# lvrcek/GNNome-assembly

Measured on AMD Instinct MI355X. Metric: GatedGCN edges/sec fwd+bwd, chr19 assembly graph, higher is better.
Workload: dtype f32 (f16x2 split products, f32 accumulate)

## Files before the change

### gnnome_assembly_amd/csrc/gnm_fused.hip

```cpp
#include <string.h>
#include <type_traits>

#include "gnm_common.h"
#include "gnm_tr.h"

namespace gnm {

typedef float floatx16 __attribute__((ext_vector_type(16)));

constexpr int FH = 128;
constexpr int FTR = 64;
constexpr int FP = FH + 4;
constexpr int FKQ = FH / 8;

using full_t = std::true_type;
using ragged_t = std::false_type;

__global__ void pack_w_k(const float* __restrict__ W, int64_t ld, int ncb, int nn, float* __restrict__ Wp) {
  const int total = ncb * FKQ * 64;
  for (int idx = blockIdx.x * blockDim.x + threadIdx.x; idx < total; idx += gridDim.x * blockDim.x) {
    const int lane = idx & 63, q = (idx >> 6) % FKQ, cb = idx / (64 * FKQ);
    const int i = lane & 31, g = lane >> 5;
    float v[4];
#pragma unroll
// ... 210 lines not shown
    for (int c = 0; c < BKC; ++c) {
      h16x8 n0[2], n1[2];
#pragma unroll
      for (int s = 0; s < 2; ++s) {
        n0[s] = a0[s];
        n1[s] = a1[s];
        if (c + 1 < BKC) {
          n0[s] = *reinterpret_cast<const h16x8*>(p0 + s * BIMG + 16 * (c + 1));
          n1[s] = *reinterpret_cast<const h16x8*>(p1 + s * BIMG + 16 * (c + 1));
        }
      }
      __builtin_amdgcn_sched_barrier(0);
      mfh(acc0, a0[1], f.w[c][0]); mfh(acc1, a1[1], f.w[c][0]);
      mfh(acc0, a0[0], f.w[c][1]); mfh(acc1, a1[0], f.w[c][1]);
      mfh(acc0, a0[0], f.w[c][0]); mfh(acc1, a1[0], f.w[c][0]);
#pragma unroll
      for (int s = 0; s < 2; ++s) { a0[s] = n0[s]; a1[s] = n1[s]; }
      __builtin_amdgcn_sched_barrier(0);
    }
  }
};

template <class MM>
__device__ __forceinline__ float stage_row(void* img, int row, int c4, const float4& v) {
  if constexpr (MM::kScaled) return MM::stage(img, row, c4, v);
  else { MM::stage(img, row, c4, v); return 1.f; }
}

__device__ __forceinline__ void h2_stage_nn(void* img, int row, int c4, const float4& v, int* eref, float* fs, bool first,
                                            bool writer) {
  const unsigned mb = row32_max_bits(max_abs4_bits(v));
  int e = (int)(mb >> 23) & 0xff;
  e = e < 16 ? 16 : e;
  const int eo = first ? e : *eref;
  const int en = e > eo ? e : eo;
  if (writer) {
    *eref = en;
    const int fe = 127 + eo - en;
    *fs = __int_as_float((fe < 0 ? 0 : fe) << 23);
  }
  h16x4 hi, lo;
  split2(v, __int_as_float((268 - en) << 23), hi, lo);
  _Float16* b = reinterpret_cast<_Float16*>(img) + row * BP + c4;
  *reinterpret_cast<h16x4*>(b) = hi;
  *reinterpret_cast<h16x4*>(b + BIMG) = lo;
}
__device__ __forceinline__ void acc_rescale_rows(floatx16& acc, const float* fs, int lg) {
#pragma unroll
  for (int q = 0; q < 4; ++q) {
    const float4 f = ld4(fs + 8 * q + 4 * lg);
    acc[4 * q + 0] *= f.x; acc[4 * q + 1] *= f.y; acc[4 * q + 2] *= f.z; acc[4 * q + 3] *= f.w;
  }
}
__device__ __forceinline__ float h2_ref_inv(int eref) { return __int_as_float((eref - 14) << 23); }

__device__ __forceinline__ void mma32_h2(const void* img, int row0, const MmH2::Frag& f, floatx16& acc, int li, int lg) {
  const _Float16* p0 = reinterpret_cast<const _Float16*>(img) + (row0 + li) * BP + 8 * lg;
#pragma unroll
  for (int c = 0; c < BKC; ++c) {
    h16x8 a0[2];
#pragma unroll
    for (int s = 0; s < 2; ++s) a0[s] = *reinterpret_cast<const h16x8*>(p0 + s * BIMG + 16 * c);
    mfh(acc, a0[1], f.w[c][0]);
    mfh(acc, a0[0], f.w[c][1]);
    mfh(acc, a0[0], f.w[c][0]);
    __builtin_amdgcn_sched_barrier(0);
  }
}

__device__ __forceinline__ void h2_stage_row64(void* img, int row, int c4, const float4& v, float* rinv_slot, bool writer) {
  unsigned m = row32_max_bits(max_abs4_bits(v));
  const unsigned o = (unsigned)__shfl_xor((int)m, 32);
  m = o > m ? o : m;
  float sc, inv;
  h2_scale(m, sc, inv);
  if (writer) *rinv_slot = inv;
  h16x4 hi, lo;
  split2(v, sc, hi, lo);
  _Float16* b = reinterpret_cast<_Float16*>(img) + row * BP + c4;
  *reinterpret_cast<h16x4*>(b) = hi;
  *reinterpret_cast<h16x4*>(b + BIMG) = lo;
}

template <class MM>
__device__ __forceinline__ void tn_store_slab(float* __restrict__ sl, const floatx16 (&tn)[2][2], int wn, int wc,
                                              int li, int lg) {
#pragma unroll
  for (int a = 0; a < 2; ++a)
#pragma unroll
    for (int b = 0; b < 2; ++b)
#pragma unroll
      for (int e = 0; e < 16; ++e) {
        const int i = (e & 3) + 8 * (e >> 2) + 4 * lg;
        const int n = (2 * wn + a) * 32 + i;
        const int c = (2 * wc + b) * 32 + li;
        sl[n * FH + c] = tn[a][b][e];
      }
}

__device__ __forceinline__ void mma32_b3(const void* img, int row0, const MmB3::Frag& f, floatx16& acc, int li, int lg) {
  const __bf16* p0 = reinterpret_cast<const __bf16*>(img) + (row0 + li) * BP + 8 * lg;
#pragma unroll
  for (int c = 0; c < BKC; ++c) {
    bf16x8 a0[3];
#pragma unroll
    for (int s = 0; s < 3; ++s) a0[s] = *reinterpret_cast<const bf16x8*>(p0 + s * BIMG + 16 * c);
    mfb(acc, a0[2], f.w[c][0]);
    mfb(acc, a0[0], f.w[c][2]);
    mfb(acc, a0[1], f.w[c][1]);
    mfb(acc, a0[1], f.w[c][0]);
    mfb(acc, a0[0], f.w[c][1]);
    mfb(acc, a0[0], f.w[c][0]);
    __builtin_amdgcn_sched_barrier(0);
  }
}

__global__ void pack_w3_k(const float* __restrict__ W, int64_t ld, int ncb, int nn, bf16x8* __restrict__ Wp) {
  const int total = ncb * BKC * 64;
  for (int idx = blockIdx.x * blockDim.x + threadIdx.x; idx < total; idx += gridDim.x * blockDim.x) {
    const int lane = idx & 63, c = (idx >> 6) % BKC, cb = idx / (64 * BKC);
    const int i = lane & 31, g = lane >> 5;
    bf16x8 hi, mid, lo;
#pragma unroll
    for (int j = 0; j < 8; ++j) {
      const int k = 16 * c + 8 * g + j;
      const float x = nn ? W[(int64_t)k * ld + cb * 32 + i] : W[(int64_t)(cb * 32 + i) * ld + k];
      const __bf16 h = (__bf16)x;
      const float r1 = x - (float)h;
      const __bf16 m = (__bf16)r1;
      hi[j] = h;
      mid[j] = m;
      lo[j] = (__bf16)(r1 - (float)m);
    }
    bf16x8* o = Wp + ((int64_t)(cb * BKC + c) * 3) * 64 + lane;
    o[0] = hi;
    o[64] = mid;
    o[128] = lo;
  }
}

static void launch_pack_w2_gen(const float* W, int64_t ld, int ncls, int ncg, int nn, void* ws, hipStream_t st);

static int g_matmul_mode = 2;
constexpr size_t kPackBytesPerBlk = MmB3::kPackBytes;

template <class MM>
static void launch_pack(const float* W, int64_t ld, int ncb, int nn, void* wp, hipStream_t st) {
  if (MM::kScaled) launch_pack_w2_gen(W, ld, ncb / 4, 1, nn, wp, st);
  else if (MM::kSplit) hipLaunchKernelGGL(pack_w3_k, dim3(4 * ncb), dim3(256), 0, st, W, ld, ncb, nn, (bf16x8*)wp);
  else hipLaunchKernelGGL(pack_w_k, dim3(4 * ncb), dim3(256), 0, st, W, ld, ncb, nn, (float*)wp);
}

template <class MM, bool EDGE, int NCG>
__global__ __launch_bounds__(kBlock, ((MM::kSplit && !EDGE && NCG == 1) || (EDGE && !MM::kSplit)) ? 2 : 1) void rowtile_nt_k(
    int64_t M, const float* __restrict__ X, const void* __restrict__ Wp, const float* __restrict__ bias,
    float* __restrict__ Y, int64_t ldy, const float* __restrict__ P,
    const int32_t* __restrict__ isrc, const int32_t* __restrict__ idst, double* __restrict__ partials,
    int64_t tiles_per_block, int ncgs) {
  __shared__ __attribute__((aligned(16))) unsigned char xraw[MM::kImgBytes];
  constexpr bool INPLACE = EDGE || NCG == 1;
  __shared__ float ys[INPLACE ? 4 : FTR * FP];
  __shared__ int sd[2 * FTR];
  float* xs = reinterpret_cast<float*>(xraw);
  const int tid = threadIdx.x, lane = tid & 63;
  const int wave = __builtin_amdgcn_readfirstlane(tid >> 6);
  const int li = lane & 31, lg = lane >> 5;
  int chunk = xcd_chunk(blockIdx.x, gridDim.x), cgb = 0;
  if (ncgs > 1) {
    const int xcd = blockIdx.x % kXcds, j = blockIdx.x / kXcds;
    cgb = j % ncgs;
    chunk = xcd * (gridDim.x / ncgs / kXcds) + j / ncgs;
  }
  const int64_t ntiles = (M + FTR - 1) / FTR;
  const int64_t tb0 = (int64_t)chunk * tiles_per_block;
  const int64_t tb1 = min(ntiles, tb0 + tiles_per_block);
  const int64_t nfull = min(tb1, M / FTR);
  const int lrow = tid >> 5, lc4 = (tid & 31) * 4;
  const int64_t Mlast = M - 1;

  typename MM::Frag wf;
  auto load_w = [&](int cg) __attribute__((always_inline)) { MM::load_w(wf, Wp, (cgb + cg) * 4 + wave, lane); };
  constexpr int ncg = NCG;
  if (ncg == 1) load_w(0);

  float4 pre[8];
  int pre_idx = 0;
  auto prefetch = [&](int64_t tile) __attribute__((always_inline)) {
    const int64_t r0 = tile * FTR;
#pragma unroll
    for (int it = 0; it < 8; ++it) {
      const float* px = X + clampi(r0 + lrow + 8 * it, Mlast) * FH + lc4;
      pre[it] = EDGE ? ld4_nt(px) : ld4(px);
    }
    if (EDGE) {
      const int64_t r = clampi(r0 + (tid & (FTR - 1)), Mlast);
      pre_idx = (tid & FTR) ? idst[r] : isrc[r];
    }
  };

  Stat4 st;
  st.zero();
  auto body = [&](auto tag, int64_t tile) __attribute__((always_inline)) {
    constexpr bool FULL = decltype(tag)::value;
    float rsc[8];
    __syncthreads();
#pragma unroll
    for (int it = 0; it < 8; ++it) rsc[it] = stage_row<MM>(xraw, lrow + 8 * it, lc4, pre[it]);
    if (EDGE && tid < 2 * FTR) sd[tid] = pre_idx;
    __syncthreads();
    const int64_t r0 = tile * FTR;
    constexpr bool LATE = EDGE && !MM::kSplit;
    float4 g1[8], g2[8];
    if (EDGE && !LATE) {
#pragma unroll
      for (int it = 0; it < 8; ++it) {
        const int row = lrow + 8 * it;
        const int64_t s_ = sd[row], d_ = sd[FTR + row];
        g1[it] = ld4(P + s_ * (5 * FH) + 3 * FH + lc4);
        g2[it] = ld4(P + d_ * (5 * FH) + 4 * FH + lc4);
      }
    }
    prefetch(tile + 1 < tb1 ? tile + 1 : tile);
#pragma unroll
    for (int cg = 0; cg < ncg; ++cg) {
      if (ncg > 1) load_w(cg);
      floatx16 acc0, acc1;
#pragma unroll
      for (int e = 0; e < 16; ++e) { acc0[e] = 0.f; acc1[e] = 0.f; }
      MM::mma(xraw, wf, acc0, acc1, li, lg);
      if (LATE) {
#pragma unroll
        for (int it = 0; it < 8; ++it) {
          const int row = lrow + 8 * it;
          const int64_t s_ = sd[row], d_ = sd[FTR + row];
          g1[it] = ld4(P + s_ * (5 * FH) + 3 * FH + lc4);
          g2[it] = ld4(P + d_ * (5 * FH) + 4 * FH + lc4);
        }
      }
      float* os = INPLACE ? xs : ys;
      if (INPLACE) __syncthreads();
      else if (cg > 0) __syncthreads();
      acc_to_lds(os, acc0, acc1, wave, li, lg);
      __syncthreads();
      const float4 b4 = ld4(bias + (cgb + cg) * FH + lc4);
      float4 ci4 = f4(1.f);
      if constexpr (MM::kScaled) ci4 = MM::col_inv4(Wp, (cgb + cg) * 4, lc4);
#pragma unroll
      for (int it = 0; it < 8; ++it) {
        const int row = lrow + 8 * it;
        const int64_t grow = r0 + row;
        float4 v = ld4(os + row * FP + lc4);
        if constexpr (MM::kScaled) v = v * (ci4 * rsc[it]);
        v = v + b4;
        if (EDGE) v = v + g1[it] + g2[it];
        if (FULL || grow < M) {
          if (EDGE) st4_nt(Y + grow * ldy + (cgb + cg) * FH + lc4, v);
          else st4(Y + grow * ldy + (cgb + cg) * FH + lc4, v);
          if (EDGE) st.add_prod(v, v);
        }
      }
    }
  };

  if (tb0 < tb1) prefetch(tb0);
  if (tb0 < nfull) {
#pragma unroll
    for (int it = 0; it < 8; ++it) st4(Y + (tb0 * FTR + lrow + 8 * it) * ldy + cgb * FH + lc4, f4(0.f));
    for (int64_t tile = tb0; tile < nfull; ++tile) body(full_t{}, tile);
  }
  if (nfull < tb1 && nfull >= tb0) body(ragged_t{}, nfull);
  if (EDGE) {
    __syncthreads();
    block_stat_store<FH>(st, reinterpret_cast<double*>(xs), partials, chunk);
  }
}

constexpr int ER3 = 32;
template <class MM>
__global__ __launch_bounds__(kBlock, 2) void edge_t32_b3p_k(
    int64_t M, const float* __restrict__ X, const void* __restrict__ Wp, const float* __restrict__ bias,
    float* __restrict__ Y, const float* __restrict__ P, const int32_t* __restrict__ isrc,
    const int32_t* __restrict__ idst, double* __restrict__ partials, int64_t tiles_per_block) {
  __shared__ __attribute__((aligned(16))) unsigned char xraw[MM::kImgBytes];
  __shared__ float os[ER3 * FP];
  __shared__ int sd[2][2 * ER3];
  const int tid = threadIdx.x, lane = tid & 63;
  const int wave = __builtin_amdgcn_readfirstlane(tid >> 6);
  const int li = lane & 31, lg = lane >> 5;
  const int chunk = xcd_chunk(blockIdx.x, gridDim.x);
  const int64_t ntiles = (M + ER3 - 1) / ER3;
  const int64_t tb0 = (int64_t)chunk * tiles_per_block;
  const int64_t tb1 = min(ntiles, tb0 + tiles_per_block);
  const int64_t nfull = min(tb1, M / ER3);
  const int lrow = tid >> 5, lc4 = (tid & 31) * 4;
  const int64_t Mlast = M - 1;
  const int32_t* const ibase = (lane & 32) ? idst : isrc;

  typename MM::Frag wf;
  MM::load_w(wf, Wp, wave, lane);
  const float4 b4 = ld4(bias + lc4);
  float4 ci4 = f4(1.f);
  if constexpr (MM::kScaled) ci4 = MM::col_inv4(Wp, 0, lc4);
  float rsc[2][4];
  float4 pre[2][4];
  int pidx[2] = {0, 0};
  auto prefetch = [&](float4 (&buf)[4], int& idx, int64_t tile) __attribute__((always_inline)) {
    const int64_t r0 = (tile < tb1 ? tile : tb1 - 1) * ER3;
#pragma unroll
    for (int it = 0; it < 4; ++it) buf[it] = ld4_nt(X + clampi(r0 + lrow + 8 * it, Mlast) * FH + lc4);
    idx = ibase[clampi(r0 + (lane & 31), Mlast)];
  };
  Stat4 st;
  st.zero();
  auto body = [&](auto tag, float4 (&nbuf)[4], int& nidx, int64_t tile, int hb) __attribute__((always_inline)) {
    constexpr bool FULL = decltype(tag)::value;
    const int64_t r0 = tile * ER3;
    float4 g1[4], g2[4];
#pragma unroll
    for (int it = 0; it < 4; ++it) {
      const int row = lrow + 8 * it;
      const int64_t s_ = sd[hb][row], d_ = sd[hb][ER3 + row];
      g1[it] = ld4(P + s_ * (5 * FH) + 3 * FH + lc4);
      g2[it] = ld4(P + d_ * (5 * FH) + 4 * FH + lc4);
    }
    floatx16 acc;
#pragma unroll
    for (int e = 0; e < 16; ++e) acc[e] = 0.f;
    if constexpr (MM::kScaled) {
      const _Float16* p0 = reinterpret_cast<const _Float16*>(xraw) + (32 * hb + li) * BP + 8 * lg;
#pragma unroll
      for (int c = 0; c < BKC; ++c) {
        h16x8 a0[2];
#pragma unroll
        for (int s_ = 0; s_ < 2; ++s_) a0[s_] = *reinterpret_cast<const h16x8*>(p0 + s_ * BIMG + 16 * c);
        mfh(acc, a0[1], wf.w[c][0]);
        if (c < 4) rsc[hb ^ 1][c] = MM::stage(xraw, 32 * (hb ^ 1) + lrow + 8 * c, lc4, nbuf[c]);
        mfh(acc, a0[0], wf.w[c][1]);
        mfh(acc, a0[0], wf.w[c][0]);
        __builtin_amdgcn_sched_barrier(0);
      }
    } else {
      const __bf16* p0 = reinterpret_cast<const __bf16*>(xraw) + (32 * hb + li) * BP + 8 * lg;
#pragma unroll
      for (int c = 0; c < BKC; ++c) {
        bf16x8 a0[3];
#pragma unroll
        for (int s_ = 0; s_ < 3; ++s_) a0[s_] = *reinterpret_cast<const bf16x8*>(p0 + s_ * BIMG + 16 * c);
        mfb(acc, a0[2], wf.w[c][0]);
        mfb(acc, a0[0], wf.w[c][2]);
        mfb(acc, a0[1], wf.w[c][1]);
        if (c < 4) MM::stage(xraw, 32 * (hb ^ 1) + lrow + 8 * c, lc4, nbuf[c]);
        mfb(acc, a0[1], wf.w[c][0]);
        mfb(acc, a0[0], wf.w[c][1]);
        mfb(acc, a0[0], wf.w[c][0]);
        __builtin_amdgcn_sched_barrier(0);
      }
    }
    sd[hb ^ 1][lane] = nidx;
    prefetch(nbuf, nidx, tile + 3);
    __syncthreads();
#pragma unroll
    for (int e = 0; e < 16; ++e) os[((e & 3) + 8 * (e >> 2) + 4 * lg) * FP + wave * 32 + li] = acc[e];
    __syncthreads();
#pragma unroll
    for (int it = 0; it < 4; ++it) {
      const int row = lrow + 8 * it;
      const int64_t grow = r0 + row;
      float4 v = ld4(os + row * FP + lc4);
      if constexpr (MM::kScaled) v = v * (ci4 * rsc[hb][it]);
      v = v + b4 + g1[it] + g2[it];
      if (FULL || grow < M) {
        st4_nt(Y + grow * FH + lc4, v);
        st.add_prod(v, v);
      }
    }
  };
  if (tb0 < tb1) {
    prefetch(pre[0], pidx[0], tb0);
    prefetch(pre[1], pidx[1], tb0 + 1);
#pragma unroll
    for (int it = 0; it < 4; ++it) rsc[0][it] = stage_row<MM>(xraw, lrow + 8 * it, lc4, pre[0][it]);
    sd[0][lane] = pidx[0];
    prefetch(pre[0], pidx[0], tb0 + 2);
    __syncthreads();
  }
  int64_t tile = tb0;
  for (; tile + 2 <= nfull; tile += 2) {
    body(full_t{}, pre[1], pidx[1], tile, 0);
    body(full_t{}, pre[0], pidx[0], tile + 1, 1);
  }
  int hb = 0;
  for (; tile < tb1; ++tile, hb ^= 1) {
    if (hb == 0) body(ragged_t{}, pre[1], pidx[1], tile, 0);
    else body(ragged_t{}, pre[0], pidx[0], tile, 1);
  }
  __syncthreads();
  block_stat_store<FH>(st, reinterpret_cast<double*>(xraw), partials, chunk);
}

constexpr int WH = 2 * FH;
constexpr int kBlockW = 512;
template <class MM>
__global__ __launch_bounds__(kBlockW, 1) void edge_t32_h256p_k(
    int64_t M, const float* __restrict__ X, const void* __restrict__ Wp, const float* __restrict__ bias,
    float* __restrict__ Y, const float* __restrict__ P, const int32_t* __restrict__ isrc,
    const int32_t* __restrict__ idst, double* __restrict__ partials, int nchunk, int64_t tiles_per_chunk) {
  __shared__ __attribute__((aligned(16))) unsigned char xraw[2 * MM::kImgBytes];
  __shared__ float os[2 * ER3 * FP];
  __shared__ int sd[2][2 * ER3];
  __shared__ float rinv[2][ER3];
  const int tid = threadIdx.x, lane = tid & 63;
  const int wave = __builtin_amdgcn_readfirstlane(tid >> 6);
  const int li = lane & 31, lg = lane >> 5;
  const int cb = wave & 3, kh = wave >> 2;
  const int xcd = blockIdx.x % kXcds, jj = blockIdx.x / kXcds;
  const int J = jj & 1, chunk = xcd * (nchunk / kXcds) + (jj >> 1);
  const int64_t ntiles = (M + ER3 - 1) / ER3;
  const int64_t tb0 = (int64_t)chunk * tiles_per_chunk;
  const int64_t tb1 = min(ntiles, tb0 + tiles_per_chunk);
  const int64_t nfull = min(tb1, M / ER3);
  const int srow = tid >> 6, sc = (tid & 63) * 4;
  unsigned char* const simg = xraw + (sc >> 7) * MM::kImgBytes;
  const int slc4 = sc & (FH - 1);
  const int erow = tid >> 5, ec4 = (tid & 31) * 4;
  const int64_t Mlast = M - 1;
  const int32_t* const ibase = (lane & 32) ? idst : isrc;

  typename MM::Frag wf;
  MM::load_w(wf, Wp, (J * 2 + kh) * 4 + cb, lane);
  const float4 b4 = ld4(bias + J * FH + ec4);
  float4 ci4 = f4(1.f);
  if constexpr (MM::kScaled) ci4 = MM::col_inv4(Wp, J * 2 * 4, ec4);
  auto stage = [&](int buf, int r, const float4& v) __attribute__((always_inline)) {
    if constexpr (MM::kScaled) h2_stage_row64(simg, 32 * buf + r, slc4, v, &rinv[buf][r], (tid & 63) == 0);
    else MM::stage(simg, 32 * buf + r, slc4, v);
  };
  float4 pre[2][4];
  int pidx[2] = {0, 0};
  auto prefetch = [&](float4 (&buf)[4], int& idx, int64_t tile) __attribute__((always_inline)) {
    const int64_t r0 = (tile < tb1 ? tile : tb1 - 1) * ER3;
#pragma unroll
    for (int it = 0; it < 4; ++it) buf[it] = ld4(X + clampi(r0 + srow + 8 * it, Mlast) * WH + sc);
    idx = ibase[clampi(r0 + (lane & 31), Mlast)];
  };
  Stat4 st;
  st.zero();
  auto body = [&](auto tag, float4 (&nbuf)[4], int& nidx, int64_t tile, int hb) __attribute__((always_inline)) {
    constexpr bool FULL = decltype(tag)::value;
    const int64_t r0 = tile * ER3;
    floatx16 acc;
#pragma unroll
    for (int e = 0; e < 16; ++e) acc[e] = 0.f;
    float ri[2] = {1.f, 1.f};
    if constexpr (MM::kScaled) { ri[0] = rinv[hb][erow]; ri[1] = rinv[hb][erow + 16]; }
    if constexpr (MM::kScaled) {
      const _Float16* p0 = reinterpret_cast<const _Float16*>(xraw + kh * MM::kImgBytes) + (32 * hb + li) * BP + 8 * lg;
      h16x8 a0[2];
#pragma unroll
      for (int s_ = 0; s_ < 2; ++s_) a0[s_] = *reinterpret_cast<const h16x8*>(p0 + s_ * BIMG);
#pragma unroll
      for (int c = 0; c < BKC; ++c) {
        h16x8 n0[2];
#pragma unroll
        for (int s_ = 0; s_ < 2; ++s_) n0[s_] = c + 1 < BKC ? *reinterpret_cast<const h16x8*>(p0 + s_ * BIMG + 16 * (c + 1)) : a0[s_];
        __builtin_amdgcn_sched_barrier(0);
        mfh(acc, a0[1], wf.w[c][0]);
        if (c < 4) stage(hb ^ 1, srow + 8 * c, nbuf[c]);
        mfh(acc, a0[0], wf.w[c][1]);
        mfh(acc, a0[0], wf.w[c][0]);
#pragma unroll
        for (int s_ = 0; s_ < 2; ++s_) a0[s_] = n0[s_];
        __builtin_amdgcn_sched_barrier(0);
      }
    } else {
      const __bf16* p0 = reinterpret_cast<const __bf16*>(xraw + kh * MM::kImgBytes) + (32 * hb + li) * BP + 8 * lg;
      bf16x8 a0[3];
#pragma unroll
      for (int s_ = 0; s_ < 3; ++s_) a0[s_] = *reinterpret_cast<const bf16x8*>(p0 + s_ * BIMG);
#pragma unroll
      for (int c = 0; c < BKC; ++c) {
        bf16x8 n0[3];
#pragma unroll
        for (int s_ = 0; s_ < 3; ++s_) n0[s_] = c + 1 < BKC ? *reinterpret_cast<const bf16x8*>(p0 + s_ * BIMG + 16 * (c + 1)) : a0[s_];
        __builtin_amdgcn_sched_barrier(0);
        mfb(acc, a0[2], wf.w[c][0]);
        mfb(acc, a0[0], wf.w[c][2]);
        mfb(acc, a0[1], wf.w[c][1]);
        if (c < 4) stage(hb ^ 1, srow + 8 * c, nbuf[c]);
        mfb(acc, a0[1], wf.w[c][0]);
        mfb(acc, a0[0], wf.w[c][1]);
        mfb(acc, a0[0], wf.w[c][0]);
#pragma unroll
        for (int s_ = 0; s_ < 3; ++s_) a0[s_] = n0[s_];
        __builtin_amdgcn_sched_barrier(0);
      }
    }
    float4 g1[2], g2[2];
#pragma unroll
    for (int it = 0; it < 2; ++it) {
      const int row = erow + 16 * it;
      const int64_t s_ = sd[hb][row], d_ = sd[hb][ER3 + row];
      g1[it] = ld4(P + s_ * (5 * WH) + 3 * WH + J * FH + ec4);
      g2[it] = ld4(P + d_ * (5 * WH) + 4 * WH + J * FH + ec4);
    }
    if (wave == 0) sd[hb ^ 1][lane] = nidx;
    prefetch(nbuf, nidx, tile + 3);
    __syncthreads();
    float* const oh = os + kh * (ER3 * FP);
#pragma unroll
    for (int e = 0; e < 16; ++e) oh[((e & 3) + 8 * (e >> 2) + 4 * lg) * FP + cb * 32 + li] = acc[e];
    __syncthreads();
#pragma unroll
    for (int it = 0; it < 2; ++it) {
      const int row = erow + 16 * it;
      const int64_t grow = r0 + row;
      float4 v = ld4(os + row * FP + ec4) + ld4(os + ER3 * FP + row * FP + ec4);
      if constexpr (MM::kScaled) v = v * (ci4 * ri[it]);
      v = v + b4 + g1[it] + g2[it];
      if (FULL || grow < M) {
        st4_nt(Y + grow * WH + J * FH + ec4, v);
        st.add_prod(v, v);
      }
    }
  };
  if (tb0 < tb1) {
    prefetch(pre[0], pidx[0], tb0);
    prefetch(pre[1], pidx[1], tb0 + 1);
#pragma unroll
    for (int it = 0; it < 4; ++it) stage(0, srow + 8 * it, pre[0][it]);
    if (wave == 0) sd[0][lane] = pidx[0];
    prefetch(pre[0], pidx[0], tb0 + 2);
    __syncthreads();
  }
  int64_t tile = tb0;
  for (; tile + 2 <= nfull; tile += 2) {
    body(full_t{}, pre[1], pidx[1], tile, 0);
    body(full_t{}, pre[0], pidx[0], tile + 1, 1);
  }
  int hb = 0;
  for (; tile < tb1; ++tile, hb ^= 1) {
    if (hb == 0) body(ragged_t{}, pre[1], pidx[1], tile, 0);
    else body(ragged_t{}, pre[0], pidx[0], tile, 1);
  }
  __syncthreads();
#pragma unroll
  for (int i = 0; i < 4; ++i) {
    st.a[i] += __shfl_xor(st.a[i], 32, 64);
    st.b[i] += __shfl_xor(st.b[i], 32, 64);
  }
  double* red = reinterpret_cast<double*>(xraw);
// ... 740 lines not shown
  static_assert(!MM::kSplit, "the split mode has its own weight-gradient kernel (tn_tr_k)");
  __shared__ __attribute__((aligned(16))) unsigned char raw[MM::kTnBytes];
  float* as = reinterpret_cast<float*>(raw);
  float* bs = as + FTR * FP;
  const int tid = threadIdx.x, lane = tid & 63;
  const int wave = __builtin_amdgcn_readfirstlane(tid >> 6);
  const int li = lane & 31, lg = lane >> 5;
  const int wn = wave >> 1, wc = wave & 1;
  const int xcd = blockIdx.x % kXcds, j = blockIdx.x / kXcds;
  const int cg = j % ncg, slot = xcd * (nslot / kXcds) + j / ncg;
  const int64_t ntiles = (M + FTR - 1) / FTR;
  const int64_t tb0 = (int64_t)slot * tiles_per_slot;
  const int64_t tb1 = min(ntiles, tb0 + tiles_per_slot);
  const int lrow = tid >> 5, lc4 = (tid & 31) * 4;
  const int64_t Mlast = M - 1;
  floatx16 tn[2][2];
#pragma unroll
  for (int a = 0; a < 2; ++a)
#pragma unroll
    for (int b = 0; b < 2; ++b)
#pragma unroll
      for (int e = 0; e < 16; ++e) tn[a][b][e] = 0.f;
  double c0 = 0.0, c1 = 0.0, c2 = 0.0, c3 = 0.0;
  constexpr int DEPTH = 1;
  float4 pa[DEPTH][8], pb[DEPTH][8];
  auto prefetch = [&](float4 (&qa)[8], float4 (&qb)[8], int64_t tile) __attribute__((always_inline)) {
    const int64_t r0 = (tile < tb1 ? tile : tb1 - 1) * FTR;
#pragma unroll
    for (int it = 0; it < 8; ++it) {
      const int64_t r = clampi(r0 + MM::row(lrow, it), Mlast);
      qa[it] = ld4(A + r * lda + cg * FH + lc4);
      qb[it] = ld4(B + r * FH + lc4);
    }
  };
  auto step = [&](float4 (&qa)[8], float4 (&qb)[8], int64_t tile) __attribute__((always_inline)) {
    const int64_t r0 = tile * FTR;
    __syncthreads();
#pragma unroll
    for (int it = 0; it < 8; ++it) {
      const bool ok = r0 + MM::row(lrow, it) < M;
      if (!ok) qa[it] = f4(0.f);
      const float4 av = qa[it];
      c0 += (double)av.x; c1 += (double)av.y; c2 += (double)av.z; c3 += (double)av.w;
      st4(as + MM::row(lrow, it) * FP + lc4, av);
      st4(bs + MM::row(lrow, it) * FP + lc4, qb[it]);
    }
    __syncthreads();
    prefetch(qa, qb, tile + DEPTH);
    mma_tn64(as, bs, tn, wn, wc, li, lg);
  };
  if (tb0 < tb1) {
#pragma unroll
    for (int d = 0; d < DEPTH; ++d) prefetch(pa[d], pb[d], tb0 + d);
    int64_t tile = tb0;
    for (; tile + DEPTH <= tb1; tile += DEPTH) {
#pragma unroll
      for (int d = 0; d < DEPTH; ++d) step(pa[d], pb[d], tile + d);
    }
    if (DEPTH == 2 && tile < tb1) step(pa[0], pb[0], tile);
  }
  float* sl = slab + (size_t)(cg * nslot + slot) * FH * FH;
  tn_store_slab<MM>(sl, tn, wn, wc, li, lg);
  __syncthreads();
  double* red = reinterpret_cast<double*>(raw);
  red[lrow * FH + lc4 + 0] = c0;
  red[lrow * FH + lc4 + 1] = c1;
  red[lrow * FH + lc4 + 2] = c2;
  red[lrow * FH + lc4 + 3] = c3;
  __syncthreads();
  if (tid < FH) {
    double s_ = 0.0;
#pragma unroll
    for (int k = 0; k < 8; ++k) s_ += red[k * FH + tid];
    partials[(size_t)(cg * nslot + slot) * FH + tid] = s_;
  }
}

__global__ __launch_bounds__(256) void slab_reduce_k(const float* __restrict__ slab, int nslab, int total, float* __restrict__ out) {
  __shared__ __attribute__((aligned(16))) float red[8 * 128];
  slab += (size_t)blockIdx.y * nslab * total;
  out += (size_t)blockIdx.y * total;
  const int i0 = blockIdx.x * 128;
  const float4 s_ = slab_reduce_128(slab, nslab, total, i0, red);
  if (threadIdx.x < 32) st4(out + i0 + threadIdx.x * 4, s_);
}

__global__ __launch_bounds__(256) void slab_reduce_ld_k(const float* __restrict__ slab, int nslab, int ncgb, float* __restrict__ out, int64_t ldc) {
  __shared__ __attribute__((aligned(16))) float red[8 * 128];
  const int m = blockIdx.x, cls = blockIdx.y;
  slab += (size_t)cls * nslab * FH * FH;
  out += (int64_t)(cls / ncgb) * FH * ldc + (cls % ncgb) * FH;
  const float4 s_ = slab_reduce_128(slab, nslab, FH * FH, m * FH, red);
  if (threadIdx.x < 32) st4(out + (int64_t)m * ldc + threadIdx.x * 4, s_);
}

}

using namespace gnm;

static inline int64_t cdiv_(int64_t a, int64_t b) { return (a + b - 1) / b; }

namespace gnm {
int tn_tr_rows_per_tile();
int tn_tr_occupancy(bool conv = false, bool h2 = false);
void tn_tr_launch(int64_t M, const float* A, int64_t lda, int ncg, const void* B, int64_t ldb, int ncgb, float* slab,
                  double* partials, int nslot, int64_t tiles_per_slot, hipStream_t st, const TnConv* cv = nullptr, bool h2 = false);
size_t edge_bwd_tr_pack_bytes();
int edge_bwd_tr_launch(int64_t E, const float* ge, float* ge_out, const float* t, const float* e_in, const float* stat_e,
                       const float* bstat_e, const float* gamma_e, const float* W3, void* wpack, float* slab,
                       double* partials, hipStream_t st, bool h2 = false, bool given = false);
}
static int g_eb_variant = 1;
static int g_gate2_wg = 2;
namespace gnm {
int eb_variant() { return g_eb_variant; }
int gate2_wg() { return g_gate2_wg; }
}
extern "C" int gnm_debug_set_variant(const char* what, int v) {
  if (what && !strcmp(what, "edge_bwd")) { g_eb_variant = v; return 0; }
  if (what && !strcmp(what, "gate2_wg") && (v == 1 || v == 2)) { g_gate2_wg = v; return 0; }
  ::gnm::set_error("debug_set_variant: unknown switch");
  return -1;
}


extern "C" size_t gnm_rowtile_workspace_bytes(int ncols) { return (size_t)(ncols / 32) * kPackBytesPerBlk; }

extern "C" int gnm_set_matmul_mode(int mode) {
  GNM_CHECK_ARG(mode >= 0 && mode <= 2, "set_matmul_mode: mode %d (0 = fp32 MFMA, 1 = bf16x3 split, 2 = f16x2 split)", mode);
  g_matmul_mode = mode;
  return 0;
}
extern "C" int gnm_get_matmul_mode(void) { return g_matmul_mode; }

template <class MM>
static int edge_t_fused_impl(int64_t E, const float* e_in, const float* W3, const float* b3, const float* P,
                             const int32_t* isrc, const int32_t* idst, float* t, double* partials, int* nblk_out,
                             void* ws, void* stream) {
  hipStream_t st = (hipStream_t)stream;
  launch_pack<MM>(W3, FH, FH / 32, 0, ws, st);
  GNM_LAUNCH_CHECK("pack_w (NT)");
  if constexpr (MM::kSplit) {
    const int64_t ntiles = cdiv_(E, ER3);
    const int grid = persistent_grid(ntiles, 8, occ_blocks<edge_t32_b3p_k<MM>>());
    hipLaunchKernelGGL(edge_t32_b3p_k<MM>, dim3(grid), dim3(kBlock), 0, st, E, e_in, (const void*)ws, b3, t, P, isrc, idst,
                       partials, cdiv_(ntiles, grid));
    GNM_LAUNCH_CHECK("edge_t_fused_fwd");
    *nblk_out = grid;
    return 0;
  }
  const int64_t ntiles = cdiv_(E, FTR);
  const int grid = persistent_grid(ntiles, 4, occ_blocks<rowtile_nt_k<MM, true, 1>>());
  hipLaunchKernelGGL((rowtile_nt_k<MM, true, 1>), dim3(grid), dim3(kBlock), 0, st, E, e_in, (const void*)ws, b3, t,
                     (int64_t)FH, P, isrc, idst, partials, cdiv_(ntiles, grid), 1);
  GNM_LAUNCH_CHECK("edge_t_fused_fwd");
  *nblk_out = grid;
  return 0;
}

extern "C" int gnm_edge_t_fused_fwd(int64_t E, int H, const float* e_in, const float* W3, const float* b3,
                                    const float* P, const int32_t* isrc, const int32_t* idst, float* t,
                                    double* partials, int* nblk_out, void* ws, size_t ws_bytes, void* stream) {
  GNM_CHECK_ARG(H == FH || (H == WH && g_matmul_mode), "edge_t_fused_fwd: H=%d (128, and 256 in the split matmul modes, are built)", H);
  GNM_CHECK_ARG(E > 0 && e_in && W3 && b3 && P && isrc && idst && t && partials && nblk_out, "edge_t_fused_fwd: null/neg argument");
  if (H == WH) {
    GNM_CHECK_ARG(ws && ws_bytes >= (size_t)16 * MmB3::kPackBytes, "edge_t_fused_fwd: workspace too small");
    hipStream_t st = (hipStream_t)stream;
    const bool h2 = g_matmul_mode == 2;
    if (h2) launch_pack_w2_gen(W3, (int64_t)WH, 2, 2, 0, ws, st);
    else hipLaunchKernelGGL(pack_w3_gen_k, dim3(64), dim3(256), 0, st, W3, (int64_t)WH, 2, 2, 0, (bf16x8*)ws);
    GNM_LAUNCH_CHECK("pack_w3_gen (NT 256)");
    const int64_t ntiles = cdiv_(E, ER3);
    int nchunk = num_cus() / 2 / kXcds * kXcds;
    if (nchunk < kXcds) nchunk = kXcds;
    if (nchunk > kMaxPartialBlocks) nchunk = kMaxPartialBlocks / kXcds * kXcds;
    if (h2) hipLaunchKernelGGL(edge_t32_h256p_k<MmH2>, dim3(nchunk * 2), dim3(kBlockW), 0, st, E, e_in, (const void*)ws, b3, t, P, isrc, idst,
                               partials, nchunk, cdiv_(ntiles, nchunk));
    else hipLaunchKernelGGL(edge_t32_h256p_k<MmB3>, dim3(nchunk * 2), dim3(kBlockW), 0, st, E, e_in, (const void*)ws, b3, t, P, isrc, idst,
                            partials, nchunk, cdiv_(ntiles, nchunk));
    GNM_LAUNCH_CHECK("edge_t_fused_fwd (256)");
    *nblk_out = nchunk;
    return 0;
  }
  GNM_CHECK_ARG(ws && ws_bytes >= gnm_rowtile_workspace_bytes(FH), "edge_t_fused_fwd: workspace too small");
  return g_matmul_mode == 2 ? edge_t_fused_impl<MmH2>(E, e_in, W3, b3, P, isrc, idst, t, partials, nblk_out, ws, stream)
         : g_matmul_mode  ? edge_t_fused_impl<MmB3>(E, e_in, W3, b3, P, isrc, idst, t, partials, nblk_out, ws, stream)
                          : edge_t_fused_impl<MmF32>(E, e_in, W3, b3, P, isrc, idst, t, partials, nblk_out, ws, stream);
}

extern "C" int gnm_edge_bwd_gt_nn(int64_t E, int H, const float* ge, const float* t, const float* stat_e, const float* bstat_e,
                                  const float* gamma_e, const float* W3, float* gt, float* ge_out, void* ws, size_t ws_bytes,
                                  void* stream) {
  GNM_CHECK_ARG(H == WH && g_matmul_mode, "edge_bwd_gt_nn: H=%d (256 in the split matmul modes is what is built)", H);
  GNM_CHECK_ARG(E > 0 && ge && t && stat_e && bstat_e && gamma_e && W3 && gt && ge_out && ge_out != ge && gt != ge,
                "edge_bwd_gt_nn: null / aliased argument (ge_out and gt must not be ge)");
  GNM_CHECK_ARG(ws && ws_bytes >= (size_t)16 * MmB3::kPackBytes, "edge_bwd_gt_nn: workspace too small");
  hipStream_t st = (hipStream_t)stream;
  const bool h2 = g_matmul_mode == 2;
  if (h2) launch_pack_w2_gen(W3, (int64_t)WH, 2, 2, 1, ws, st);
  else hipLaunchKernelGGL(pack_w3_gen_k, dim3(64), dim3(256), 0, st, W3, (int64_t)WH, 2, 2, 1, (bf16x8*)ws);
  GNM_LAUNCH_CHECK("pack_w3_gen (NN 256)");
  const int64_t ntiles = cdiv_(E, ER3);
  int nchunk = num_cus() / 2 / kXcds * kXcds;
  if (nchunk < kXcds) nchunk = kXcds;
  if (h2) hipLaunchKernelGGL(edge_gt_nn_h256_k<MmH2>, dim3(nchunk * 2), dim3(kBlockW), 0, st, E, ge, t, stat_e, bstat_e, gamma_e, (const void*)ws,
                             gt, ge_out, nchunk, cdiv_(ntiles, nchunk));
  else hipLaunchKernelGGL(edge_gt_nn_h256_k<MmB3>, dim3(nchunk * 2), dim3(kBlockW), 0, st, E, ge, t, stat_e, bstat_e, gamma_e, (const void*)ws,
                          gt, ge_out, nchunk, cdiv_(ntiles, nchunk));
  GNM_LAUNCH_CHECK("edge_bwd_gt_nn");
  return 0;
}

template <class MM>
static int node_proj_fwd_impl(int64_t N, int ncols, const float* h, const float* W, const float* b, float* Pout,
                              void* ws, void* stream) {
  hipStream_t st = (hipStream_t)stream;
  launch_pack<MM>(W, FH, ncols / 32, 0, ws, st);
  GNM_LAUNCH_CHECK("pack_w (NT, node)");
  const int64_t ntiles = cdiv_(N, FTR);
  if constexpr (MM::kSplit) {
    const int ncg = ncols / FH;
    int nslot = (num_cus() * occ_blocks<rowtile_nt_k<MM, false, 1>>()) / ncg / kXcds * kXcds;
    if (nslot > (int)((ntiles + kXcds - 1) / kXcds * kXcds)) nslot = (int)((ntiles + kXcds - 1) / kXcds * kXcds);
    if (nslot < kXcds) nslot = kXcds;
    hipLaunchKernelGGL((rowtile_nt_k<MM, false, 1>), dim3(nslot * ncg), dim3(kBlock), 0, st, N, h, (const void*)ws, b,
                       Pout, (int64_t)ncols, (const float*)nullptr, (const int32_t*)nullptr,
                       (const int32_t*)nullptr, (double*)nullptr, cdiv_(ntiles, nslot), ncg);
  } else {
    const int grid = persistent_grid(ntiles, 2, occ_blocks<rowtile_nt_k<MM, false, 5>>());
    hipLaunchKernelGGL((rowtile_nt_k<MM, false, 5>), dim3(grid), dim3(kBlock), 0, st, N, h, (const void*)ws, b, Pout,
                       (int64_t)ncols, (const float*)nullptr, (const int32_t*)nullptr,
                       (const int32_t*)nullptr, (double*)nullptr, cdiv_(ntiles, grid), 1);
  }
  GNM_LAUNCH_CHECK("node_proj_fwd");
  return 0;
}

extern "C" int gnm_node_proj_fwd(int64_t N, int H, int ncols, const float* h, const float* W, const float* b,
                                 float* Pout, void* ws, size_t ws_bytes, void* stream) {
  GNM_CHECK_ARG(H == FH, "node_proj_fwd: H=%d (only 128 is built)", H);
  GNM_CHECK_ARG(N > 0 && ncols == 5 * FH && h && W && b && Pout, "node_proj_fwd: bad argument (ncols must be 5*128)");
  GNM_CHECK_ARG(ws && ws_bytes >= gnm_rowtile_workspace_bytes(ncols), "node_proj_fwd: workspace too small");
  return g_matmul_mode == 2 ? node_proj_fwd_impl<MmH2>(N, ncols, h, W, b, Pout, ws, stream)
         : g_matmul_mode  ? node_proj_fwd_impl<MmB3>(N, ncols, h, W, b, Pout, ws, stream)
                          : node_proj_fwd_impl<MmF32>(N, ncols, h, W, b, Pout, ws, stream);
}

namespace gnm {
int edge_bwd_chain_launch(const ChainArgs& in, const float* W3, void* wpack, hipStream_t st, bool h2 = false);
}
extern "C" size_t gnm_edge_bwd_fused_workspace_bytes(void);

static int edge_bwd_chain_impl(int64_t N, int64_t E, int H, const float* ge, float* ge_out, const float* t_hi,
                               const float* e_mid, const float* stat_hi, const float* bstat_hi, const float* gamma_hi,
                               const float* W3_hi, float* gW3_hi, float* gb3_hi, double* partials_hi,
                               const float* t_lo, const float* stat_lo, const float* P_lo, const float* Q_lo,
                               const float* hf_lo, const float* hb_lo, const int32_t* isrc, const int32_t* idst,
                               const int32_t* in_ptr, float* gP_lo, float* Ud_lo, float* Td_lo, double* partials_lo,
                               const uint32_t* sinfo, int64_t plan_nodes_per_block, float* UT_lo,
                               int* nblk_out, void* ws, size_t ws_bytes, void* stream) {
  GNM_CHECK_ARG(H == FH, "edge_bwd_chain: H=%d (only 128 is built)", H);
  GNM_CHECK_ARG(g_matmul_mode >= 1, "edge_bwd_chain: only built for the split matmul modes");
  GNM_CHECK_ARG(N > 0 && E > 0 && ge && ge_out && t_hi && e_mid && stat_hi && bstat_hi && gamma_hi && W3_hi && gW3_hi &&
                    gb3_hi && partials_hi && t_lo && stat_lo && P_lo && Q_lo && hf_lo && hb_lo && isrc && idst && in_ptr &&
                    gP_lo && Ud_lo && Td_lo && partials_lo && nblk_out && partials_hi != partials_lo,
                "edge_bwd_chain: null / aliased argument");
  GNM_CHECK_ARG(ws && ws_bytes >= gnm_edge_bwd_fused_workspace_bytes(), "edge_bwd_chain: workspace %zu < %zu", ws_bytes,
                gnm_edge_bwd_fused_workspace_bytes());
  hipStream_t st = (hipStream_t)stream;
  float* slab = (float*)((char*)ws + gnm_rowtile_workspace_bytes(FH));
  ChainArgs a{};
  a.E = E; a.N = N;
  a.ge = ge; a.ge_out = ge_out; a.t_hi = t_hi; a.e_mid = e_mid;
  a.stat_hi = stat_hi; a.bstat_hi = bstat_hi; a.gamma_hi = gamma_hi;
  a.slab = slab; a.partials = partials_hi;
  a.t_lo = t_lo; a.stat_lo = stat_lo; a.P_lo = P_lo; a.Q_lo = Q_lo; a.hf_lo = hf_lo; a.hb_lo = hb_lo;
  a.isrc = isrc; a.idst = idst; a.in_ptr = in_ptr;
  a.gP_lo = gP_lo; a.Ud_lo = Ud_lo; a.Td_lo = Td_lo; a.partials_lo = partials_lo;
  a.sinfo = sinfo; a.UT_lo = UT_lo; a.margin = kSweepMargin;
  a.ud_pitch = Td_lo == Ud_lo + FH ? 2 * FH : FH;
  int64_t npb = 0;
  gnm_sweep_partition(N, 1, &npb, nullptr);
  GNM_CHECK_ARG((npb + 2 * kSweepMargin) * 5 * FH * 4 < (int64_t)INT32_MAX, "edge_bwd_chain: %lld nodes per workgroup exceed the 32-bit buffer offsets",
                (long long)npb);
  if (sinfo) {
    GNM_CHECK_ARG(UT_lo, "edge_bwd_chain_src: UT_lo is null");
    GNM_CHECK_ARG(plan_nodes_per_block == npb, "edge_bwd_chain_src: the sweep plan was built for %lld nodes per workgroup, the kernel uses %lld "
                  "(gnm_sweep_partition(N, 1))", (long long)plan_nodes_per_block, (long long)npb);
  }
  const int grid = edge_bwd_chain_launch(a, W3_hi, ws, st, g_matmul_mode == 2);
  GNM_LAUNCH_CHECK("edge_bwd_chain");
  hipLaunchKernelGGL(slab_reduce_k, dim3(FH * FH / 128), dim3(256), 0, st, (const float*)slab, grid, FH * FH, gW3_hi);
  GNM_LAUNCH_CHECK("edge_bwd_chain slab reduce");
  *nblk_out = grid;
  return gnm_reduce_partials(partials_hi, grid, 1, FH, gb3_hi, stream) ? -3 : 0;
}

extern "C" int gnm_edge_bwd_top(int64_t N, int64_t E, int H, float* ge, const float* e_out, const float* t,
                                const float* stat_e, const float* P, const float* Q, const float* hf, const float* hb,
                                const int32_t* isrc, const int32_t* idst, const int32_t* in_ptr, float* gP, float* Ud,
                                float* Td, double* partials, const uint32_t* sinfo, int64_t plan_nodes_per_block,
                                float* UT, int* nblk_out, void* ws, size_t ws_bytes, void* stream) {
  GNM_CHECK_ARG(H == FH || (H == 2 * FH && sinfo), "edge_bwd_top: H=%d (128; 256 with a sweep plan, one sweep per 128-column half)", H);
  GNM_CHECK_ARG(N > 0 && E > 0 && ge && e_out && t && stat_e && P && Q && hf && hb && isrc && idst && in_ptr && gP && Ud &&
                    Td && partials && nblk_out && (!sinfo || UT), "edge_bwd_top: null argument");
  GNM_CHECK_ARG(ws && ws_bytes >= gnm_edge_bwd_fused_workspace_bytes(), "edge_bwd_top: workspace %zu < %zu", ws_bytes,
                gnm_edge_bwd_fused_workspace_bytes());
  int64_t npb = 0;
  gnm_sweep_partition(N, 1, &npb, nullptr);
  GNM_CHECK_ARG((npb + 2 * kSweepMargin) * 5 * H * 4 < (int64_t)INT32_MAX, "edge_bwd_top: %lld nodes per workgroup exceed the 32-bit buffer offsets",
                (long long)npb);
  GNM_CHECK_ARG(!sinfo || plan_nodes_per_block == npb, "edge_bwd_top: the sweep plan was built for %lld nodes per workgroup, the kernel uses %lld",
                (long long)plan_nodes_per_block, (long long)npb);
  for (int c0 = 0; c0 < H; c0 += FH) {
    ChainArgs a{};
    a.E = E; a.N = N; a.hfull = H;
    a.ge = ge + c0; a.ge_out = ge + c0; a.e_mid = e_out + c0;
    a.slab = (float*)((char*)ws + gnm_rowtile_workspace_bytes(FH));
    a.t_lo = t + c0; a.stat_lo = stat_e + c0; a.P_lo = P + c0; a.Q_lo = Q + c0; a.hf_lo = hf + c0; a.hb_lo = hb + c0;
    a.isrc = isrc; a.idst = idst; a.in_ptr = in_ptr;
    a.gP_lo = gP + c0; a.Ud_lo = Ud + c0; a.Td_lo = Td + c0; a.partials_lo = partials + c0;
    a.sinfo = sinfo; a.UT_lo = UT ? UT + c0 : nullptr; a.margin = kSweepMargin;
    a.ud_pitch = Td == Ud + H ? 2 * H : H;
    const int g = edge_bwd_chain_launch(a, nullptr, nullptr, (hipStream_t)stream);
    GNM_CHECK_ARG(g > 0, "edge_bwd_top: no kernel for this configuration");
    *nblk_out = g;
    GNM_LAUNCH_CHECK("edge_bwd_top");
  }
  return 0;
}

extern "C" int gnm_ln_edge_bwd_top(int64_t N, int64_t E, int H, float* ge, const float* e_out, const float* t, const float* gamma_e,
                                   const float* beta_e, int width, const float* P, const float* Q, const float* hf, const float* hb,
                                   const int32_t* isrc, const int32_t* idst, const int32_t* in_ptr, float* gP, float* gt,
                                   double* partials, const uint32_t* sinfo, int64_t plan_nodes_per_block, int* nblk_out, void* ws,
                                   size_t ws_bytes, void* stream) {
  GNM_CHECK_ARG(H == FH, "ln_edge_bwd_top: H=%d (only 128 is built)", H);
  GNM_CHECK_ARG(width >= 1 && width <= H, "ln_edge_bwd_top: width must be in [1, H]");
  GNM_CHECK_ARG(N > 0 && E > 0 && ge && e_out && t && gamma_e && beta_e && P && Q && hf && hb && isrc && idst && in_ptr && gP && gt &&
                    partials && sinfo && nblk_out, "ln_edge_bwd_top: null argument");
  GNM_CHECK_ARG(ws && ws_bytes >= gnm_edge_bwd_fused_workspace_bytes(), "ln_edge_bwd_top: workspace %zu < %zu", ws_bytes,
                gnm_edge_bwd_fused_workspace_bytes());
  int64_t npb = 0;
  gnm_sweep_partition(N, 1, &npb, nullptr);
  GNM_CHECK_ARG((npb + 2 * kSweepMargin) * 5 * H * 4 < (int64_t)INT32_MAX, "ln_edge_bwd_top: %lld nodes per workgroup exceed the 32-bit buffer offsets",
                (long long)npb);
  GNM_CHECK_ARG(plan_nodes_per_block == npb, "ln_edge_bwd_top: the sweep plan was built for %lld nodes per workgroup, the kernel uses %lld",
                (long long)plan_nodes_per_block, (long long)npb);
  ChainArgs a{};
  a.E = E; a.N = N; a.hfull = H;
  a.ge = ge; a.ge_out = ge; a.e_mid = e_out;
  a.slab = (float*)((char*)ws + gnm_rowtile_workspace_bytes(FH));
  a.t_lo = t; a.P_lo = P; a.Q_lo = Q; a.q_pitch = 4 * H; a.qb_off = 2 * H; a.hf_lo = hf; a.hb_lo = hb;
  a.isrc = isrc; a.idst = idst; a.in_ptr = in_ptr;
  a.gP_lo = gP; a.Ud_lo = gP + 4 * H; a.Td_lo = gP + 4 * H; a.ud_pitch = 5 * H;
  a.UT_lo = gP + 3 * H; a.ut_pitch = 5 * H;
  a.partials_lo = partials;
  a.sinfo = sinfo; a.margin = kSweepMargin;
  a.ln_gamma = gamma_e; a.ln_beta = beta_e; a.ln_width = width; a.gt_out = gt;
  const int g = edge_bwd_chain_launch(a, nullptr, nullptr, (hipStream_t)stream);
  GNM_CHECK_ARG(g > 0, "ln_edge_bwd_top: no kernel for this configuration");
  *nblk_out = g;
  GNM_LAUNCH_CHECK("ln_edge_bwd_top");
  return 0;
}

extern "C" int gnm_ln_edge_bwd_chain(int64_t N, int64_t E, int H, float* ge, const float* gt_hi, const float* e_mid, const float* W3_hi,
                                     float* gW3_hi, float* gb3_hi, double* partials_hi, const float* t_lo, const float* gamma_lo,
                                     const float* beta_lo, int width, const float* P_lo, const float* Q_lo, const float* hf_lo,
                                     const float* hb_lo, const int32_t* isrc, const int32_t* idst, const int32_t* in_ptr, float* gP_lo,
                                     float* gt_lo, double* partials_lo, const uint32_t* sinfo, int64_t plan_nodes_per_block,
                                     int* nblk_out, void* ws, size_t ws_bytes, void* stream) {
  GNM_CHECK_ARG(H == FH, "ln_edge_bwd_chain: H=%d (only 128 is built)", H);
  GNM_CHECK_ARG(g_matmul_mode >= 1, "ln_edge_bwd_chain: only built for the split matmul modes");
  GNM_CHECK_ARG(width >= 1 && width <= H, "ln_edge_bwd_chain: width must be in [1, H]");
  GNM_CHECK_ARG(N > 0 && E > 0 && ge && gt_hi && e_mid && W3_hi && gW3_hi && gb3_hi && partials_hi && t_lo && gamma_lo && beta_lo && P_lo &&
                    Q_lo && hf_lo && hb_lo && isrc && idst && in_ptr && gP_lo && gt_lo && partials_lo && sinfo && nblk_out &&
                    partials_hi != partials_lo && gt_hi != gt_lo, "ln_edge_bwd_chain: null / aliased argument");
  GNM_CHECK_ARG(ws && ws_bytes >= gnm_edge_bwd_fused_workspace_bytes(), "ln_edge_bwd_chain: workspace %zu < %zu", ws_bytes,
                gnm_edge_bwd_fused_workspace_bytes());
  hipStream_t st = (hipStream_t)stream;
  float* slab = (float*)((char*)ws + gnm_rowtile_workspace_bytes(FH));
  int64_t npb = 0;
  gnm_sweep_partition(N, 1, &npb, nullptr);
  GNM_CHECK_ARG((npb + 2 * kSweepMargin) * 5 * FH * 4 < (int64_t)INT32_MAX, "ln_edge_bwd_chain: %lld nodes per workgroup exceed the 32-bit buffer offsets",
// ... 318 lines not shown
```

Baseline: 47.97 million.

## Add dedicated 32-row split-matmul kernel for node projection forward

Replaces the generic 64-row rowtile kernel for the split-precision node projection with a specialised kernel. The new kernel uses 32-row tiles, double-buffered staging interleaved with the MFMA loop, and a small LDS output tile, and splits each team across column groups. The generic kernel loses its column-group parameter and the occupancy-2 case for node projections. Smaller tiles aim for better occupancy and load balance on the node matmul, at the cost of more per-tile overhead and more syncs.

```diff
diff --git a/gnnome_assembly_amd/csrc/gnm_fused.hip b/gnnome_assembly_amd/csrc/gnm_fused.hip
--- a/gnnome_assembly_amd/csrc/gnm_fused.hip
+++ b/gnnome_assembly_amd/csrc/gnm_fused.hip
@@ -386,11 +386,11 @@
 }
 
 template <class MM, bool EDGE, int NCG>
-__global__ __launch_bounds__(kBlock, ((MM::kSplit && !EDGE && NCG == 1) || (EDGE && !MM::kSplit)) ? 2 : 1) void rowtile_nt_k(
+__global__ __launch_bounds__(kBlock, (EDGE && !MM::kSplit) ? 2 : 1) void rowtile_nt_k(
     int64_t M, const float* __restrict__ X, const void* __restrict__ Wp, const float* __restrict__ bias,
     float* __restrict__ Y, int64_t ldy, const float* __restrict__ P,
     const int32_t* __restrict__ isrc, const int32_t* __restrict__ idst, double* __restrict__ partials,
-    int64_t tiles_per_block, int ncgs) {
+    int64_t tiles_per_block) {
   __shared__ __attribute__((aligned(16))) unsigned char xraw[MM::kImgBytes];
   constexpr bool INPLACE = EDGE || NCG == 1;
   __shared__ float ys[INPLACE ? 4 : FTR * FP];
@@ -399,12 +399,8 @@
   const int tid = threadIdx.x, lane = tid & 63;
   const int wave = __builtin_amdgcn_readfirstlane(tid >> 6);
   const int li = lane & 31, lg = lane >> 5;
-  int chunk = xcd_chunk(blockIdx.x, gridDim.x), cgb = 0;
-  if (ncgs > 1) {
-    const int xcd = blockIdx.x % kXcds, j = blockIdx.x / kXcds;
-    cgb = j % ncgs;
-    chunk = xcd * (gridDim.x / ncgs / kXcds) + j / ncgs;
-  }
+  const int chunk = xcd_chunk(blockIdx.x, gridDim.x);
+  constexpr int cgb = 0;
   const int64_t ntiles = (M + FTR - 1) / FTR;
   const int64_t tb0 = (int64_t)chunk * tiles_per_block;
   const int64_t tb1 = min(ntiles, tb0 + tiles_per_block);
@@ -630,6 +626,105 @@
   }
   __syncthreads();
   block_stat_store<FH>(st, reinterpret_cast<double*>(xraw), partials, chunk);
+}
+
+template <class MM>
+__global__ __launch_bounds__(kBlock, 2) void node_t32_p_k(
+    int64_t M, const float* __restrict__ X, const void* __restrict__ Wp, const float* __restrict__ bias,
+    float* __restrict__ Y, int ncgs, int64_t tiles_per_team) {
+  __shared__ __attribute__((aligned(16))) unsigned char xraw[MM::kImgBytes];
+  __shared__ float os[ER3 * FP];
+  const int tid = threadIdx.x, lane = tid & 63;
+  const int wave = __builtin_amdgcn_readfirstlane(tid >> 6);
+  const int li = lane & 31, lg = lane >> 5;
+  const int lrow = tid >> 5, lc4 = (tid & 31) * 4;
+  const int64_t ldy = (int64_t)ncgs * FH;
+  const int64_t ntiles = (M + ER3 - 1) / ER3, Mlast = M - 1;
+  const int xcd = blockIdx.x % kXcds, j = blockIdx.x / kXcds;
+  const int cgb = j % ncgs, team = xcd * (gridDim.x / ncgs / kXcds) + j / ncgs;
+  const int64_t tb0 = (int64_t)team * tiles_per_team;
+  const int64_t tb1 = min(ntiles, tb0 + tiles_per_team);
+  if (tb0 >= tb1) return;
+  const int64_t nfull = min(tb1, M / ER3);
+  typename MM::Frag wf;
+  MM::load_w(wf, Wp, cgb * 4 + wave, lane);
+  const float4 b4 = ld4(bias + cgb * FH + lc4);
+  float4 ci4 = f4(1.f);
+  if constexpr (MM::kScaled) ci4 = MM::col_inv4(Wp, cgb * 4, lc4);
+  float rsc[2][4];
+  float4 pre[2][4];
+  auto prefetch = [&](float4 (&buf)[4], int64_t tile) __attribute__((always_inline)) {
+    const int64_t t0 = (tile < tb1 ? tile : tb1 - 1) * ER3;
+#pragma unroll
+    for (int it = 0; it < 4; ++it) buf[it] = ld4(X + clampi(t0 + lrow + 8 * it, Mlast) * FH + lc4);
+  };
+  auto body = [&](auto tag, float4 (&nbuf)[4], int64_t tile, int hb) __attribute__((always_inline)) {
+    constexpr bool FULL = decltype(tag)::value;
+    const int64_t t0 = tile * ER3;
+    floatx16 acc;
+#pragma unroll
+    for (int e = 0; e < 16; ++e) acc[e] = 0.f;
+    if constexpr (MM::kScaled) {
+      const _Float16* p0 = reinterpret_cast<const _Float16*>(xraw) + (32 * hb + li) * BP + 8 * lg;
+#pragma unroll
+      for (int c = 0; c < BKC; ++c) {
+        h16x8 a0[2];
+#pragma unroll
+        for (int s_ = 0; s_ < 2; ++s_) a0[s_] = *reinterpret_cast<const h16x8*>(p0 + s_ * BIMG + 16 * c);
+        mfh(acc, a0[1], wf.w[c][0]);
+        if (c < 4) rsc[hb ^ 1][c] = MM::stage(xraw, 32 * (hb ^ 1) + lrow + 8 * c, lc4, nbuf[c]);
+        mfh(acc, a0[0], wf.w[c][1]);
+        mfh(acc, a0[0], wf.w[c][0]);
+        __builtin_amdgcn_sched_barrier(0);
+      }
+    } else {
+      const __bf16* p0 = reinterpret_cast<const __bf16*>(xraw) + (32 * hb + li) * BP + 8 * lg;
+#pragma unroll
+      for (int c = 0; c < BKC; ++c) {
+        bf16x8 a0[3];
+#pragma unroll
+        for (int s_ = 0; s_ < 3; ++s_) a0[s_] = *reinterpret_cast<const bf16x8*>(p0 + s_ * BIMG + 16 * c);
+        mfb(acc, a0[2], wf.w[c][0]);
+        mfb(acc, a0[0], wf.w[c][2]);
+        mfb(acc, a0[1], wf.w[c][1]);
+        if (c < 4) MM::stage(xraw, 32 * (hb ^ 1) + lrow + 8 * c, lc4, nbuf[c]);
+        mfb(acc, a0[1], wf.w[c][0]);
+        mfb(acc, a0[0], wf.w[c][1]);
+        mfb(acc, a0[0], wf.w[c][0]);
+        __builtin_amdgcn_sched_barrier(0);
+      }
+    }
+    prefetch(nbuf, tile + 3);
+    __syncthreads();
+#pragma unroll
+    for (int e = 0; e < 16; ++e) os[((e & 3) + 8 * (e >> 2) + 4 * lg) * FP + wave * 32 + li] = acc[e];
+    __syncthreads();
+#pragma unroll
+    for (int it = 0; it < 4; ++it) {
+      const int row = lrow + 8 * it;
+      const int64_t grow = t0 + row;
+      float4 v = ld4(os + row * FP + lc4);
+      if constexpr (MM::kScaled) v = v * (ci4 * rsc[hb][it]);
+      v = v + b4;
+      if (FULL || grow < M) st4(Y + grow * ldy + cgb * FH + lc4, v);
+    }
+  };
+  prefetch(pre[0], tb0);
+  prefetch(pre[1], tb0 + 1);
+#pragma unroll
+  for (int it = 0; it < 4; ++it) rsc[0][it] = stage_row<MM>(xraw, lrow + 8 * it, lc4, pre[0][it]);
+  prefetch(pre[0], tb0 + 2);
+  __syncthreads();
+  int64_t tile = tb0;
+  for (; tile + 2 <= nfull; tile += 2) {
+    body(full_t{}, pre[1], tile, 0);
+    body(full_t{}, pre[0], tile + 1, 1);
+  }
+  int hb = 0;
+  for (; tile < tb1; ++tile, hb ^= 1) {
+    if (hb == 0) body(ragged_t{}, pre[1], tile, 0);
+    else body(ragged_t{}, pre[0], tile, 1);
+  }
 }
 
 constexpr int WH = 2 * FH;
@@ -1676,7 +1771,7 @@
   const int64_t ntiles = cdiv_(E, FTR);
   const int grid = persistent_grid(ntiles, 4, occ_blocks<rowtile_nt_k<MM, true, 1>>());
   hipLaunchKernelGGL((rowtile_nt_k<MM, true, 1>), dim3(grid), dim3(kBlock), 0, st, E, e_in, (const void*)ws, b3, t,
-                     (int64_t)FH, P, isrc, idst, partials, cdiv_(ntiles, grid), 1);
+                     (int64_t)FH, P, isrc, idst, partials, cdiv_(ntiles, grid));
   GNM_LAUNCH_CHECK("edge_t_fused_fwd");
   *nblk_out = grid;
   return 0;
@@ -1744,17 +1839,17 @@
   const int64_t ntiles = cdiv_(N, FTR);
   if constexpr (MM::kSplit) {
     const int ncg = ncols / FH;
-    int nslot = (num_cus() * occ_blocks<rowtile_nt_k<MM, false, 1>>()) / ncg / kXcds * kXcds;
-    if (nslot > (int)((ntiles + kXcds - 1) / kXcds * kXcds)) nslot = (int)((ntiles + kXcds - 1) / kXcds * kXcds);
-    if (nslot < kXcds) nslot = kXcds;
-    hipLaunchKernelGGL((rowtile_nt_k<MM, false, 1>), dim3(nslot * ncg), dim3(kBlock), 0, st, N, h, (const void*)ws, b,
-                       Pout, (int64_t)ncols, (const float*)nullptr, (const int32_t*)nullptr,
-                       (const int32_t*)nullptr, (double*)nullptr, cdiv_(ntiles, nslot), ncg);
+    const int64_t nt32 = cdiv_(N, ER3);
+    int nteam = (num_cus() * occ_blocks<node_t32_p_k<MM>>()) / ncg / kXcds * kXcds;
+    if (nteam > (int)((nt32 + kXcds - 1) / kXcds * kXcds)) nteam = (int)((nt32 + kXcds - 1) / kXcds * kXcds);
+    if (nteam < kXcds) nteam = kXcds;
+    hipLaunchKernelGGL(node_t32_p_k<MM>, dim3(nteam * ncg), dim3(kBlock), 0, st, N, h, (const void*)ws, b, Pout, ncg,
+                       cdiv_(nt32, nteam));
   } else {
     const int grid = persistent_grid(ntiles, 2, occ_blocks<rowtile_nt_k<MM, false, 5>>());
     hipLaunchKernelGGL((rowtile_nt_k<MM, false, 5>), dim3(grid), dim3(kBlock), 0, st, N, h, (const void*)ws, b, Pout,
                        (int64_t)ncols, (const float*)nullptr, (const int32_t*)nullptr,
-                       (const int32_t*)nullptr, (double*)nullptr, cdiv_(ntiles, grid), 1);
+                       (const int32_t*)nullptr, (double*)nullptr, cdiv_(ntiles, grid));
   }
   GNM_LAUNCH_CHECK("node_proj_fwd");
   return 0;
```

After: 47.86 million. About the same (-0.2%).
